# li-kunyi/dns-slam

Measured on AMD Instinct MI355X. Metric: ray-samples/s, higher is better.
Workload: dtype f32 (MLP products as 3 x f16 split-operand MFMA / 6 x bf16 for weight gradients, f32 accumulate: error <= fp32 fma chain)

## Files before the change

### dns_slam_amd/_lib.py

```python
from __future__ import annotations

import ctypes as C
import os

_HERE = os.path.dirname(os.path.abspath(__file__))
LIB_PATH = os.environ.get("DNS_HIP_LIB") or os.path.join(_HERE, "libdns_hip.so")
DNS_MAX_LEVELS = 32
ABI_VERSION = 17


class DnsGridMeta(C.Structure):
    _fields_ = [
        ("n_levels", C.c_uint32), ("n_features", C.c_uint32), ("log2_hashmap_size", C.c_uint32),
        ("base_resolution", C.c_uint32), ("total_rows", C.c_uint32), ("per_level_scale", C.c_float),
        ("scale", C.c_float * DNS_MAX_LEVELS), ("resolution", C.c_uint32 * DNS_MAX_LEVELS),
        ("size", C.c_uint32 * DNS_MAX_LEVELS), ("offset", C.c_uint32 * DNS_MAX_LEVELS),
        ("hashed", C.c_uint32 * DNS_MAX_LEVELS),
    ]


class DnsSplitRows(C.Structure):
    _fields_ = [("rows", C.c_void_p), ("exps", C.c_void_p), ("ld", C.c_uint32), ("lo_off", C.c_uint32)]


class DnsAdamTensor(C.Structure):
    _fields_ = [("p", C.c_void_p), ("g", C.c_void_p), ("m", C.c_void_p), ("v", C.c_void_p), ("n", C.c_uint64),
                ("lr", C.c_float)]


_P = C.c_void_p
_U = C.c_uint32
_I = C.c_int


class DnsTrackFused(C.Structure):
    _fields_ = [("color", _P), ("depth", _P), ("label", _P),
                ("H", C.c_int32), ("W", C.c_int32), ("H0", C.c_int32), ("H1", C.c_int32), ("W0", C.c_int32), ("W1", C.c_int32),
                ("cam", _P), ("bound", _P),
                ("pix", _P), ("t_uniform", _P), ("t_surf", _P), ("t_zero", _P), ("dmax", _P), ("iter", _P), ("n_iters", _U),
                ("n_uniform", _U), ("n_surface", _U), ("n_rays", _U),
                ("quat", _P), ("trans", _P),
                ("table", _P), ("meta", C.POINTER(DnsGridMeta)), ("n_bins", _U),
                ("w_coarse", _P), ("w_color", _P), ("w_logit", _P),
                ("n_neurons", _U), ("n_hidden_layers", _U), ("hidden", _U), ("n_feat", _U), ("n_class", _U),
                ("code", _P), ("code_dim", _U),
                ("lambda_p", C.c_float), ("lambda_d", C.c_float), ("lambda_l", C.c_float),
                ("ws", _P), ("adam_m", _P), ("adam_v", _P), ("adam_state", _P),
                ("lr_quat", C.c_float), ("lr_trans", C.c_float), ("beta1", C.c_float), ("beta2", C.c_float), ("eps", C.c_float),
                ("best_loss", _P), ("best_cam", _P), ("out", _P), ("g_quat", _P), ("g_trans", _P)]

SIGNATURES = {
# ... 40 lines not shown
    "dns_class_slots": (C.c_int, [_P, _U, _U, _I, _P, _U, _P, _P]),
    "dns_feature_block": (C.c_int, [_P, _U, _U, _P, _U, _P, _P, _U, _U, _P, _U, _P, _P]),
    "dns_rgb_sigmoid": (C.c_int, [_P, _U, _P]),
    "dns_raw_bwd": (C.c_int, [_P, _P, _U, _P, _P, _U, _I, _P]),
    "dns_lattice_points": (C.c_int, [_P, _P, _U, _P, _U, _P, _P]),
    "dns_draw_finish": (C.c_int, [_P, _P, _P, _P, _P, _P, _P, _P, _U, _U, _U, _U, _P, _P, _P, _P]),
    "dns_track_mask": (C.c_int, [_P, _P, _U, C.c_float, _P, _P]),
    "dns_keep_best": (C.c_int, [_P, _P, _P, _P, _P, _P]),
    "dns_force_half": (C.c_int, [_P, _U, _U, _P]),
    "dns_track_fused_ws_floats": (C.c_uint64, [C.POINTER(DnsTrackFused)]),
    "dns_track_fused_begin": (C.c_int, [_P, _U, _U, _P, _I, _I, _I, _I, _P, _U, _P, _P]),
    "dns_track_fused_iter": (C.c_int, [C.POINTER(DnsTrackFused), _P]),
    "dns_feature_gather": (C.c_int, [_P, _P, _P, _P, _U, _U, _U, _I, _I, _I, _I, _P, _P, _P]),
    "dns_feature_gather_frames": (C.c_int, [_P, _P, _P, _P, _P, _U, _U, _U, _U, _I, _I, _I, _I, _P, _U, _P, _P]),
    "dns_refer_poses": (C.c_int, [_P, _P, _P, _P, _U, _P, _P, _P]),
    "dns_merge_dy": (C.c_int, [_P, _U, _U, _U, _U, _P, _P, _U, _U, _P, _P]),
    "dns_add_ref_sum": (C.c_int, [_P, _U, _U, _U, _P, _P]),
    "dns_tv_fwd": (C.c_int, [_P, _U, _U, _U, _I, _U, _P, _P]),
    "dns_tv_bwd": (C.c_int, [_P, _U, _U, _U, _I, _U, _P, _P, _P]),
    "dns_group_slots": (C.c_int, [_P, _U, _U, _U, _U, _P, _P, _P, _P]),
    "dns_group_scatter": (C.c_int, [_P, _U, _U, _P, _U, _P, _P]),
    "dns_device_error": (C.c_int, [C.c_int]),
    "dns_adam_step": (C.c_int, [C.POINTER(DnsAdamTensor), _U, C.c_float, C.c_float, C.c_float, _P, _P]),
    "dns_composite_fwd": (C.c_int, [_P, _P, _P, _U, _U, _U, _P, _P, _P, _P, _P, _P]),
    "dns_composite_bwd": (C.c_int, [_P, _P, _P, _U, _U, _U, _P, _P, _P, _P, _P, _P, _P, _P]),
    "dns_mc_ws_bytes": (C.c_uint64, [_U, _U, _U]),
    "dns_mc_count": (C.c_int, [_P, _U, _U, _U, C.c_float, _P, _P, _P]),
    "dns_mc_emit": (C.c_int, [_P, _U, _U, _U, C.c_float, C.POINTER(C.c_double), C.POINTER(C.c_double), _P, _P, C.c_uint64, _P,
                              C.c_uint64, _P]),
    "dns_keyframe_project": (C.c_int, [_P, _U, _P, _U, _P, _P, _I, _I, C.POINTER(C.c_float), _P, _P, _P]),
    "dns_mesh_cc_ws_bytes": (C.c_uint64, [_U]),
    "dns_mesh_components": (C.c_int, [_P, _U, _P, _U, _P, _P, _P, _P, _P]),
    "dns_nearest_ws_bytes": (C.c_uint64, [_U, _U]),
    "dns_nearest_points": (C.c_int, [_P, _U, _P, _U, _U, _U, _P, _P, _P, _P, _P]),
    "dns_icp_ws_bytes": (C.c_uint64, [_U, _U]),
    "dns_icp_point_to_point": (C.c_int, [_P, _U, _P, _U, C.POINTER(C.c_double), C.c_float, _U, C.c_double, C.c_double, _U, _P, _P,
                                         _P, _P]),
    "dns_frustum_seen": (C.c_int, [_P, _U, _P, _U, _I, _I, C.POINTER(C.c_float), _P, _P]),
    "dns_ms_ssim_window": (None, [C.POINTER(C.c_float)]),
    "dns_ms_ssim_ws_bytes": (C.c_uint64, [_U, _U, _U]),
    "dns_ms_ssim": (C.c_int, [_P, _P, _P, _U, _U, _U, _P, _P, _P, _P, _P, _P]),
    "dns_label_confusion": (C.c_int, [_P, _P, _U, C.c_uint64, _U, _P, _P, _P]),
}


def _load():
# ... 68 lines not shown
```

### dns_slam_amd/csrc/adam.hip

```cpp
#include "common.hpp"

namespace dns {

constexpr int ADAM_MAX_TENSORS = 32;

struct AdamBatch {
  float* p[ADAM_MAX_TENSORS];
  const float* g[ADAM_MAX_TENSORS];
  float* m[ADAM_MAX_TENSORS];
  float* v[ADAM_MAX_TENSORS];
  uint32_t block_end[ADAM_MAX_TENSORS];
  uint32_t n[ADAM_MAX_TENSORS];
  float lr[ADAM_MAX_TENSORS];
  uint32_t n_tensors;
};

__global__ void adam_tick_kernel(float* __restrict__ state, float beta1, float beta2) {
  if (threadIdx.x == 0 && blockIdx.x == 0) {
    const float t = state[0] + 1.0f;
    state[0] = t;
    state[1] = 1.0f - powf(beta1, t);
    state[2] = 1.0f - powf(beta2, t);
  }
}

__global__ __launch_bounds__(256) void adam_step_kernel(AdamBatch b, const float* __restrict__ state, float beta1, float beta2,
                                                        float eps) {
  uint32_t t = 0;
  while (t + 1 < b.n_tensors && blockIdx.x >= b.block_end[t]) ++t;
  const uint32_t first = t ? b.block_end[t - 1] : 0u;
  const uint32_t i0 = (blockIdx.x - first) * 1024u + threadIdx.x * 4u;
  const uint32_t n = b.n[t];
  if (i0 >= n) return;
  const float bc1 = state[1], bc2 = state[2];
  const float step_size = b.lr[t] / bc1;
  const float inv_sqrt_bc2 = 1.0f / sqrtf(bc2);
  float* __restrict__ p = b.p[t];
  const float* __restrict__ g = b.g[t];
  float* __restrict__ m = b.m[t];
  float* __restrict__ v = b.v[t];
  const float ob1 = 1.0f - beta1, ob2 = 1.0f - beta2;
  if (i0 + 3u < n && (((uintptr_t)(p + i0) | (uintptr_t)(g + i0) | (uintptr_t)(m + i0) | (uintptr_t)(v + i0)) & 15u) == 0) {
    const float4 g4 = *reinterpret_cast<const float4*>(g + i0);
    float4 m4 = *reinterpret_cast<const float4*>(m + i0), v4 = *reinterpret_cast<const float4*>(v + i0);
    float4 p4 = *reinterpret_cast<const float4*>(p + i0);
    const float ge[4] = {g4.x, g4.y, g4.z, g4.w};
    float me[4] = {m4.x, m4.y, m4.z, m4.w}, ve[4] = {v4.x, v4.y, v4.z, v4.w}, pe[4] = {p4.x, p4.y, p4.z, p4.w};
#pragma unroll
    for (int e = 0; e < 4; ++e) {
      me[e] = beta1 * me[e] + ob1 * ge[e];
      ve[e] = beta2 * ve[e] + ob2 * ge[e] * ge[e];
      const float denom = sqrtf(ve[e]) * inv_sqrt_bc2 + eps;
      pe[e] -= step_size * (me[e] / denom);
    }
    *reinterpret_cast<float4*>(m + i0) = make_float4(me[0], me[1], me[2], me[3]);
    *reinterpret_cast<float4*>(v + i0) = make_float4(ve[0], ve[1], ve[2], ve[3]);
    *reinterpret_cast<float4*>(p + i0) = make_float4(pe[0], pe[1], pe[2], pe[3]);
    return;
  }
#pragma unroll
  for (uint32_t e = 0; e < 4; ++e) {
    const uint32_t i = i0 + e;
    if (i < n) {
      const float gi = g[i];
      const float mi = beta1 * m[i] + ob1 * gi;
      const float vi = beta2 * v[i] + ob2 * gi * gi;
      m[i] = mi;
      v[i] = vi;
      const float denom = sqrtf(vi) * inv_sqrt_bc2 + eps;
      p[i] -= step_size * (mi / denom);
    }
  }
}

}

using namespace dns;

extern "C" int dns_adam_step(const DnsAdamTensor* tensors, uint32_t n_tensors, float beta1, float beta2, float eps,
                             float* state, void* stream) {
  DNS_REQUIRE(tensors && state, "dns_adam_step: NULL argument");
  DNS_REQUIRE(n_tensors <= ADAM_MAX_TENSORS, "dns_adam_step: at most %d tensors per call (got %u)", ADAM_MAX_TENSORS, n_tensors);
  AdamBatch b;
  uint32_t nb = 0, k = 0;
  for (uint32_t i = 0; i < n_tensors; ++i) {
    if (!tensors[i].g || tensors[i].n == 0) continue;
    DNS_REQUIRE(tensors[i].p && tensors[i].m && tensors[i].v, "dns_adam_step: tensor %u has a NULL buffer", i);
    DNS_REQUIRE(tensors[i].n < (1ull << 32), "dns_adam_step: tensor %u too large", i);
    b.p[k] = tensors[i].p; b.g[k] = tensors[i].g; b.m[k] = tensors[i].m; b.v[k] = tensors[i].v;
    b.n[k] = (uint32_t)tensors[i].n;
    b.lr[k] = tensors[i].lr;
    nb += (uint32_t)((tensors[i].n + 1023) / 1024);
    b.block_end[k] = nb;
    ++k;
  }
  b.n_tensors = k;
  hipStream_t st = (hipStream_t)stream;
  DNS_LAUNCH(adam_tick_kernel, dim3(1), dim3(64), 0, st, state, beta1, beta2);
  if (k) DNS_LAUNCH(adam_step_kernel, dim3(nb), dim3(256), 0, st, b, state, beta1, beta2, eps);
  return check_launch("dns_adam_step");
}
```

### dns_slam_amd/csrc/mlp_split.hpp

```cpp
#pragma once
#include "common.hpp"
#include "split_rows.hpp"

namespace dns {
namespace sp {

typedef float f32x16 __attribute__((ext_vector_type(16)));
typedef _Float16 half8 __attribute__((ext_vector_type(8)));
typedef _Float16 half4v __attribute__((ext_vector_type(4)));

using sr::TGT_EXP;
using sr::scale_exp;

struct Frag {
  half8 hi, lo;
};

__device__ __forceinline__ uint32_t acc_row(uint32_t r, uint32_t h) { return (r & 3u) + 8u * (r >> 2) + 4u * h; }

__device__ __forceinline__ f32x16 zero16() {
  f32x16 z;
#pragma unroll
  for (int i = 0; i < 16; ++i) z[i] = 0.f;
  return z;
// ... 73 lines not shown
                                                 uint32_t lane) {
  return reinterpret_cast<const uint4*>(img) + ((rt * nsteps + s) * 2u + part) * 64u + lane;
}

template <int PREC>
__device__ __forceinline__ Frag load_frag(const _Float16* img, uint32_t nsteps, uint32_t rt, uint32_t s, uint32_t lane) {
  Frag f;
  const uint4 hi = *frag_ptr(img, nsteps, rt, s, 0, lane);
  f.hi = *reinterpret_cast<const half8*>(&hi);
  if (PREC == 3) {
    const uint4 lo = *frag_ptr(img, nsteps, rt, s, 1, lane);
    f.lo = *reinterpret_cast<const half8*>(&lo);
  } else {
    f.lo = f.hi;
  }
  return f;
}

template <int MAXQ>
struct ImgQuads {
  float4 v[MAXQ];
};

template <int MAXQ>
__device__ __forceinline__ float image_load(ImgQuads<MAXQ>& q, const float* __restrict__ M, uint32_t R, uint32_t C, uint32_t ld = 0) {
  if (ld == 0) ld = C;
  const uint32_t qpr = C >> 2, nq = R * qpr;
  const bool vec = ((((uintptr_t)M) & 15u) == 0) && ((ld & 3u) == 0);
  float m = 0.f;
  bool bad = false;
#pragma unroll
  for (int j = 0; j < MAXQ; ++j) {
    const uint32_t e = threadIdx.x + j * blockDim.x;
    q.v[j] = make_float4(0.f, 0.f, 0.f, 0.f);
    if (e < nq) {
      const uint32_t rr = e / qpr;
      const float* src = M + (size_t)rr * ld + (size_t)(e - rr * qpr) * 4u;
      if (vec) q.v[j] = *reinterpret_cast<const float4*>(src);
      else q.v[j] = make_float4(src[0], src[1], src[2], src[3]);
    }
    const float a = fmaxf(fmaxf(fabsf(q.v[j].x), fabsf(q.v[j].y)), fmaxf(fabsf(q.v[j].z), fabsf(q.v[j].w)));
    m = fmaxf(m, a);
    bad = bad || !(a < INFINITY);
  }
  return bad ? INFINITY : m;
}

template <int MAXQ>
__device__ __forceinline__ void image_scatter(const ImgQuads<MAXQ>& q, _Float16* __restrict__ img, uint32_t R, uint32_t C,
                                              bool transpose, uint32_t row_tiles, uint32_t nsteps, int kmap, float scale) {
  auto slot = [&](uint32_t i, uint32_t k, uint32_t& idx) -> bool {
    const uint32_t s = k >> 4, qq = k & 15u;
    uint32_t h, j;
    if (kmap == K_NAT) {
      h = qq >> 3;
      j = qq & 7u;
    } else {
      h = (qq >> 2) & 1u;
      j = ((qq >> 3) << 2) | (qq & 3u);
    }
    const uint32_t rt = i >> 5;
    if (rt >= row_tiles || s >= nsteps) return false;
    idx = ((((rt * nsteps + s) * 2u) * 64u) + (i & 31u) + 32u * h) * 8u + j;
    return true;
  };
  const uint32_t qpr = C >> 2, nq = R * qpr;
#pragma unroll
  for (int jq = 0; jq < MAXQ; ++jq) {
    const uint32_t e = threadIdx.x + jq * blockDim.x;
    if (e >= nq) continue;
    const uint32_t rr = e / qpr, cc = (e - rr * qpr) * 4u;
    const float vv[4] = {q.v[jq].x * scale, q.v[jq].y * scale, q.v[jq].z * scale, q.v[jq].w * scale};
    _Float16 hi[4], lo[4];
#pragma unroll
    for (int c = 0; c < 4; ++c) {
      hi[c] = (_Float16)vv[c];
      lo[c] = (_Float16)(vv[c] - (float)hi[c]);
    }
    uint32_t idx;
    if (!transpose) {
      if (slot(rr, cc, idx)) {
        half4v h4, l4;
#pragma unroll
        for (int c = 0; c < 4; ++c) { h4[c] = hi[c]; l4[c] = lo[c]; }
        *reinterpret_cast<half4v*>(img + idx) = h4;
        *reinterpret_cast<half4v*>(img + idx + 64u * 8u) = l4;
      }
    } else {
#pragma unroll
      for (uint32_t c = 0; c < 4u; ++c) {
        if (slot(cc + c, rr, idx)) {
          img[idx] = hi[c];
          img[idx + 64u * 8u] = lo[c];
        }
      }
    }
  }
}

__device__ __forceinline__ void lds_zero16(void* p, uint32_t bytes) {
  uint4* q = reinterpret_cast<uint4*>(p);
  for (uint32_t e = threadIdx.x; e < bytes / 16u; e += blockDim.x) q[e] = make_uint4(0u, 0u, 0u, 0u);
}

__device__ __forceinline__ void images_copy_in(unsigned char* lds, const unsigned char* __restrict__ src, uint32_t bytes,
                                               const unsigned char* __restrict__ exps, int* wexp) {
  const uint4* __restrict__ s4 = reinterpret_cast<const uint4*>(src);
  uint4* d4 = reinterpret_cast<uint4*>(lds);
  const uint32_t n = bytes / 16u, stride = blockDim.x;
  uint32_t e = threadIdx.x;
  for (; e + 7u * stride < n; e += 8u * stride) {
    uint4 v[8];
#pragma unroll
    for (int k = 0; k < 8; ++k) v[k] = s4[e + k * stride];
#pragma unroll
    for (int k = 0; k < 8; ++k) d4[e + k * stride] = v[k];
  }
  for (; e < n; e += stride) d4[e] = s4[e];
  if (threadIdx.x < 3) wexp[threadIdx.x] = reinterpret_cast<const int*>(exps)[threadIdx.x];
// ... 940 lines not shown
```

### dns_slam_amd/fused_step.py

```python
from __future__ import annotations

import ctypes as C
import os

import torch

from . import ops
from ._lib import DnsAdamTensor, DnsSplitRows, DnsTrackFused, check, ptr
from .common import get_quad_from_c2w, get_rotation_from_quad

_V = C.c_void_p


def _morton2(row, col):
    def spread(v):
        v = v & 0xffff
        v = (v | (v << 8)) & 0x00ff00ff
        v = (v | (v << 4)) & 0x0f0f0f0f
        v = (v | (v << 2)) & 0x33333333
        return (v | (v << 1)) & 0x55555555
    return spread(col) | (spread(row) << 1)


class _Set:
    pass


class MapStep:
    def __init__(self, mapper, target_frames, quad_list=None, T_list=None, prep=None, features=None, lambda_lt=10.0,
                 smooth=True, betas=(0.9, 0.999), eps=1e-8, keep_hidden=False, split_rows=None, refer_frames=None):
        m = self.m = mapper
# ... 120 lines not shown
        if self.half:
            self.xh = torch.empty(P, ld, device=dev, dtype=torch.float16)
            self.feath = torch.empty(P, self.n_feat, device=dev, dtype=torch.float16)
        self.use_prep = (bool(getattr(m, "prepared_images", os.environ.get("DNS_PREPARED_IMAGES", "1") != "0")) and not self.sr
                         and not self.half)
        self._blobs, self._prep_jobs = {}, []
        if self.use_prep:
            raw_lib = ops.lib._raw
            G = int(self.p_pool.shape[0]) if self.p_pool.dim() == 2 else 1
            live_n = (self.live >> 16) & 0xff
            jobs = [(self.p_coarse, self.shp_c, self.shp_c[1], 1, 0, 0),
                    (self.p_coarse, self.shp_c, 1, 1, 0, 0),
                    (self.p_pool, self.shp_f, self.shp_f[1], G, int(self.p_pool.shape[-1]), 0),
                    (self.p_color, self.shp_col, self.shp_col[1], 1, 0, self.live),
                    (self.p_logit, self.shp_log, self.shp_log[1], 1, 0, self.live)]
            for prm, shp_, n_out, n_sets, stride, lv in jobs:
                n_in_eff = live_n if lv else shp_[0]
                nfl = int(raw_lib.dns_mlp_prepared_floats(n_in_eff, n_out, shp_[2], shp_[3]))
                blob = torch.empty(nfl * n_sets + 64, device=dev)
                off = (-blob.data_ptr() // 4) % 4
                view = blob[off:off + nfl * n_sets]
                self._blobs[(prm.data_ptr(), n_out)] = view
                self._prep_jobs.append((prm, shp_[0], n_out, shp_[2], shp_[3], n_sets, stride, view, lv, blob))
        self.sr_planes = 1 if self.fp16 else 2
        self.sr_flags = 1 if self.fp16 else 0
        if self.sr:
            np_ = self.sr_planes
            h16 = lambda *s_: torch.empty(*s_, device=dev, dtype=torch.float16)
            i32 = lambda n_: torch.empty(n_, device=dev, dtype=torch.int32)
            self.xs, self.xexp = h16(P, np_ * ld), i32(P)
            self.fxs, self.fexp = h16(P, np_ * self.n_feat), i32(P)
            self.rows_x = DnsSplitRows(self.xs.data_ptr(), self.xexp.data_ptr(), np_ * ld, ld if np_ == 2 else 0)
            self.rows_f = DnsSplitRows(self.fxs.data_ptr(), self.fexp.data_ptr(), np_ * self.n_feat, self.n_feat if np_ == 2 else 0)
        nf = self.hid + 1
        self.coarse = f(P, nf)
        n_groups = self.n_groups = max(len(pool), 1)
        self.n_slots = (P + 127) // 128 * 128 + 128 * n_groups
        self.group_ws = torch.empty(512, device=dev, dtype=torch.int32)
        self.feat = f(P, self.n_feat)
        self.slot = torch.empty(P, device=dev, dtype=torch.int64)
        self.sets = []
        for _ in range(2):
            st_ = _Set()
            o_G = (P * nf + 3) // 4 * 4
            st_.zb = torch.zeros(o_G + n_G, device=dev)
            st_.fine, st_.G = st_.zb[:P * nf].view(P, nf), st_.zb[o_G:]
# ... 96 lines not shown

            code = spread(ii.reshape(-1)) | (spread(jj.reshape(-1)) << 1) | (spread(kk.reshape(-1)) << 2)
            self.lat_order_l = torch.argsort(code).contiguous()
            self.lat_order = elem[self.lat_order_l].to(torch.int32).contiguous()
            self.lat_slot = torch.empty_like(self.lat_order_l)
            self.lat_slot[self.lat_order_l] = torch.arange(Pl, device=dev)
            self.occ_x, self.d_occ_x = f(Pl, 1), f(Pl, 1)
            _, c_vox, c_off, c_mar = m._lattice_consts
            self.lat_consts = (C.c_double * 9)(*[float(v) for t in (c_vox, c_off, c_mar) for v in t.cpu().tolist()])
            self.tv = f(1)
            self.w_sm = torch.full((1,), m.lambda_sm if self.union else m.lambda_sm / self.world, device=dev)
            self.ws_mlp_l = mlp_ws(Pl, self.shp_c)
            self.h_l = f(self.shp_c[3] * Pl * self.shp_c[2]) if self.keep_h_lat else None
            self.ws_enc_l = enc_ws(Pl)
        if getattr(m, "_side_stream", None) is None:
            m._side_stream = torch.cuda.Stream(device=dev)
        self.side = m._side_stream
        self.steps = 0

    def _prepare_weights(self, st):
        for prm, n_in, n_out, nn, nl, n_sets, stride, view, lv, _ in self._prep_jobs:
            check(ops.lib.dns_mlp_prepare(ptr(prm), n_in, n_out, nn, nl, n_sets, stride, ptr(view), lv, st), "dns_mlp_prepare")

    def _w(self, params, n_out):
        blob = self._blobs.get((params.data_ptr(), n_out)) if self.use_prep else None
        if blob is None:
            return ptr(params), 0
        return ptr(blob), ops.MLP_PREPARED_FLAG

    def _lattice_branch(self, cur, st):
        lib = ops.lib
        Pl, ld, pe = self.Pl, self.ld, self.pe_dim
        pts = self.pts_l
        check(lib.dns_lattice_points(ptr(cur.draws["r6"]), self.lat_consts, self.n_lat, ptr(self.lat_order), Pl, ptr(pts), st),
              "dns_lattice_points")
        meta = C.byref(self.meta.c)
        grid_l = _V(self.bufl.data_ptr() + 4 * pe)
        n_in, _, nn, nl = self.shp_c
        if self.half:
            check(lib.dns_encode_fwd_split(ptr(pts), None, Pl, self.n_bins, ptr(self.p_table), meta, None, None, 0, ptr(self.xhl), ld,
                                           None, ops.SPLIT_PLAIN, None, st), "dns_encode_fwd_split")
            check(lib.dns_mlp_fwd_half(ptr(self.xhl), ld, None, 0, 0, ptr(self.p_coarse), n_in, 1, nn, nl, ptr(self.occ), 1, Pl,
                                       None, None, 0, 0, st), "dns_mlp_fwd_half")
        elif self.sr:
            check(lib.dns_encode_fwd_split(ptr(pts), None, Pl, self.n_bins, ptr(self.p_table), meta, None, ptr(self.bufl), ld,
                                           ptr(self.xsl), self.sr_planes * ld, ptr(self.xexpl), self.sr_flags, None, st), "dns_encode_fwd_split")
# ... 78 lines not shown
                                  ptr(self.slot), stream), "dns_class_slots")
        check(lib.dns_group_slots(ptr(self.slot), P, self.n_groups, 2, self.n_slots, ptr(self.group_ws), ptr(st_.row_index),
                                  ptr(st_.tile_group), stream), "dns_group_slots")
        st_.zb.zero_()

    @torch.no_grad()
    def step(self, draws=None, last=False):
        m, lib = self.m, ops.lib
        if torch.cuda.is_current_stream_capturing():
            self._captured = True
        main = torch.cuda.current_stream()
        st = _V(main.cuda_stream)
        K, npf, N, S, P, ld, pe = self.K, self.npf, self.N, self.S, self.P, self.ld, self.pe_dim
        prefetch = getattr(m, "prefetch_draws", False) and draws is None
        cur = self.sets[self.steps % 2]
        if not prefetch or cur.ev is None:
            self._prepare(cur, st, draws)
        else:
            main.wait_event(cur.ev)
        cur.ev = None
        self.cur = cur
        pix, (t_surf, t_zero) = cur.draws["pix"], cur.draws["jitter"]
        on_side = self.smooth and getattr(m, "overlap_smooth", False)
        if on_side or prefetch:
            self.side.wait_stream(main)
        prep_ev = None
        if self.use_prep:
            if on_side or prefetch:
                with torch.cuda.stream(self.side):
                    self._prepare_weights(_V(self.side.cuda_stream))
                    prep_ev = torch.cuda.Event()
                    prep_ev.record(self.side)
            else:
                self._prepare_weights(st)
        if on_side:
            with torch.cuda.stream(self.side):
                self._lattice_branch(cur, _V(self.side.cuda_stream))
        elif self.smooth:
            self._lattice_branch(cur, st)
        if prefetch and not last:
            nxt = self.sets[(self.steps + 1) % 2]
            with torch.cuda.stream(self.side):
                self._prepare(nxt, _V(self.side.cuda_stream), None)
                nxt.ev = torch.cuda.Event()
                nxt.ev.record(self.side)
            for t in (nxt.draws["pix"], nxt.draws["jitter"][0], nxt.draws["jitter"][1], nxt.dmax):
                t.record_stream(main)

        jstride = self.ns if t_surf.dim() == 2 else 0
        prep = self.prep
# ... 169 lines not shown
            with torch.cuda.stream(self.side):
                st2 = _V(self.side.cuda_stream)
                check(lib.dns_encode_bwd(ptr(self.x3), self.b6, P, self.n_bins, ptr(self.p_table), meta, ptr(self.d_buf), ld, d_grid,
                                         ld, None, ptr(self.d_x3), ptr(self.dydx), None, 0, 0, st2), "dns_encode_bwd")
                if self.stem:
                    check(lib.dns_add_ref_sum(ptr(self.d_rel), self.R, self.Pf, P, ptr(self.d_x3), st2), "dns_add_ref_sum")
                check(lib.dns_raygen_bwd(ptr(pix), ptr(self.Q), self.camv, 0, H, 0, W, K, npf, S, ptr(self.z), ptr(self.d_x3), None,
                                         None, ptr(self.ray_ws), ptr(cur.g_quat), ptr(cur.g_trans), st2), "dns_raygen_bwd")
        check(lib.dns_encode_bwd(ptr(self.x3), self.b6, P, self.n_bins, ptr(self.p_table), meta, ptr(self.d_buf), ld, d_grid, ld,
                                 ptr(cur.g_table), ptr(self.d_x3) if (self.is_BA and not fork_pose) else None, ptr(self.dydx),
                                 ptr(self.ws_enc), self.scatter_form, self.scatter_cap, st), "dns_encode_bwd")
        if self.is_BA and not fork_pose:
            if self.stem:
                check(lib.dns_add_ref_sum(ptr(self.d_rel), self.R, self.Pf, P, ptr(self.d_x3), st), "dns_add_ref_sum")
            check(lib.dns_raygen_bwd(ptr(pix), ptr(self.Q), self.camv, 0, H, 0, W, K, npf, S, ptr(self.z), ptr(self.d_x3), None,
                                     None, ptr(self.ray_ws), ptr(cur.g_quat), ptr(cur.g_trans), st), "dns_raygen_bwd")
        if on_side:
            main.wait_stream(self.side)
        if self.dist_on:
            import torch.distributed as dist
            work2 = dist.all_reduce(cur.G_late, op=dist.ReduceOp.SUM, group=m.dist.group, async_op=True)
            work.wait()
            work2.wait()
        check(lib.dns_adam_step(cur.adam_items, self.n_adam, self.betas[0], self.betas[1], self.eps, ptr(self.adam_state), st),
              "dns_adam_step")
        self.steps += 1

    def set_lambda_lt(self, value):
        if getattr(self, "_captured", False) and float(value) != float(self.lam[3]):
            raise RuntimeError("MapStep.set_lambda_lt: the step has been captured into a hipGraph -- the loss weights are kernel "
                               "arguments frozen at capture time; capture one graph per weight schedule phase")
        self.lam[3] = float(value)

    g_table = property(lambda self: self.cur.g_table)
    g_coarse = property(lambda self: self.cur.g_coarse)
    g_color = property(lambda self: self.cur.g_color)
    g_logit = property(lambda self: self.cur.g_logit)
    g_pool = property(lambda self: self.cur.g_pool)
    g_merge = property(lambda self: self.cur.g_merge)
    g_quat = property(lambda self: self.cur.g_quat)
    g_trans = property(lambda self: self.cur.g_trans)

    def losses(self):
        t = self.out
        terms = {"p_loss": t[0], "d_loss": t[1], "l_loss": t[2], "lt_loss": t[3], "fs_loss": t[4], "opacity_loss": t[5]}
        total = t[6]
        if self.smooth:
            terms["smooth_loss"] = self.tv[0]
# ... 386 lines not shown
```

### include/dns_hip.h

```cpp
#ifndef DNS_HIP_H
#define DNS_HIP_H

#include <stdint.h>

#ifdef __cplusplus
extern "C" {
#endif

#define DNS_ABI_VERSION 17
#define DNS_MAX_LEVELS 32

#define DNS_OK 0
#define DNS_E_ARG (-1)
#define DNS_E_LAUNCH (-2)
#define DNS_E_STATE (-3)

typedef struct DnsGridMeta {
  uint32_t n_levels;
  uint32_t n_features;
  uint32_t log2_hashmap_size;
  uint32_t base_resolution;
  uint32_t total_rows;
  float per_level_scale;
  float scale[DNS_MAX_LEVELS];
  uint32_t resolution[DNS_MAX_LEVELS];
  uint32_t size[DNS_MAX_LEVELS];
  uint32_t offset[DNS_MAX_LEVELS];
  uint32_t hashed[DNS_MAX_LEVELS];
} DnsGridMeta;

int dns_abi_version(void);
const char* dns_last_error(void);
// ... 138 lines not shown
                      const float* sums, float* out, void* stream);
int dns_loss_bwd(const float* lambdas, uint32_t N, uint32_t S, uint32_t C, uint32_t L, int tracker,
                 const float* out, const float* g_total, const float* pred_color, const float* pred_depth,
                 const float* pred_var, const float* pred_logits, const float* gt_color, const float* gt_depth,
                 const int64_t* gt_label, const uint8_t* valid, const float* fine, const float* coarse, const float* z,
                 float* d_color, float* d_depth, float* d_var, float* d_logits, float* d_fine, float* d_coarse,
                 uint32_t ldd_fine, void* stream);

int dns_loss_bwd_points(const float* lambdas, uint32_t N, uint32_t S, uint32_t C, uint32_t L, const float* out,
                        const float* g_total, const float* gt_depth, const uint8_t* valid, const float* fine, const float* coarse,
                        const float* z, float* d_fine, float* d_coarse, uint32_t ldd_fine, const float* d_occ, uint32_t ld_occ,
                        void* stream);

typedef struct DnsAdamTensor {
  float* p;
  const float* g;
  float* m;
  float* v;
  uint64_t n;
  float lr;
} DnsAdamTensor;
int dns_adam_step(const DnsAdamTensor* tensors, uint32_t n_tensors, float beta1, float beta2, float eps,
                  float* state, void* stream);

typedef struct DnsTrackFused {
  const float* color;
  const float* depth;
  const float* label;
  int32_t H, W, H0, H1, W0, W1;
  const double* cam;
  const double* bound;
  const int64_t* pix;
  const float* t_uniform;
  const float* t_surf;
  const float* t_zero;
  const uint32_t* dmax;
  uint32_t* iter;
  uint32_t n_iters;
  uint32_t n_uniform, n_surface, n_rays;
  float* quat;
  float* trans;
  const float* table;
  const DnsGridMeta* meta;
  uint32_t n_bins;
  const float* w_coarse;
  const float* w_color;
// ... 112 lines not shown
```

Measured before the change: 169.8 million.

## Fuse MLP weight image preparation into the Adam step kernel

The Adam update kernel now also rebuilds the split f16 hi/lo MFMA weight images for MLP tensors. The last block to finish each tensor, found through an atomic counter, computes the block scale exponents and scatters the forward and backward images. This removes the separate dns_mlp_prepare launches at the start of each step, which now run only when a parameter's version changes outside the optimizer. In exchange a single block serially writes all images for a tensor at the tail of the kernel, and the bias-correction tick moves into a last-block atomic.

```diff
diff --git a/dns_slam_amd/_lib.py b/dns_slam_amd/_lib.py
--- a/dns_slam_amd/_lib.py
+++ b/dns_slam_amd/_lib.py
@@ -6,7 +6,7 @@
 _HERE = os.path.dirname(os.path.abspath(__file__))
 LIB_PATH = os.environ.get("DNS_HIP_LIB") or os.path.join(_HERE, "libdns_hip.so")
 DNS_MAX_LEVELS = 32
-ABI_VERSION = 17
+ABI_VERSION = 18
 
 
 class DnsGridMeta(C.Structure):
@@ -27,6 +27,14 @@
     _fields_ = [("p", C.c_void_p), ("g", C.c_void_p), ("m", C.c_void_p), ("v", C.c_void_p), ("n", C.c_uint64),
                 ("lr", C.c_float)]
 
+
+class DnsAdamImage(C.Structure):
+    _fields_ = [("images", C.c_void_p), ("tensor", C.c_uint32), ("n_in", C.c_uint32), ("n_out", C.c_uint32),
+                ("n_neurons", C.c_uint32), ("n_hidden_layers", C.c_uint32), ("live_in", C.c_uint32), ("n_sets", C.c_uint32),
+                ("param_stride", C.c_uint32)]
+
+
+ADAM_WORK_WORDS = 33
 
 _P = C.c_void_p
 _U = C.c_uint32
@@ -113,6 +121,8 @@
     "dns_group_scatter": (C.c_int, [_P, _U, _U, _P, _U, _P, _P]),
     "dns_device_error": (C.c_int, [C.c_int]),
     "dns_adam_step": (C.c_int, [C.POINTER(DnsAdamTensor), _U, C.c_float, C.c_float, C.c_float, _P, _P]),
+    "dns_adam_step_images": (C.c_int, [C.POINTER(DnsAdamTensor), _U, C.POINTER(DnsAdamImage), _U, C.c_float, C.c_float, C.c_float,
+                                       _P, _P, _P]),
     "dns_composite_fwd": (C.c_int, [_P, _P, _P, _U, _U, _U, _P, _P, _P, _P, _P, _P]),
     "dns_composite_bwd": (C.c_int, [_P, _P, _P, _U, _U, _U, _P, _P, _P, _P, _P, _P, _P, _P]),
     "dns_mc_ws_bytes": (C.c_uint64, [_U, _U, _U]),
diff --git a/dns_slam_amd/csrc/adam.hip b/dns_slam_amd/csrc/adam.hip
--- a/dns_slam_amd/csrc/adam.hip
+++ b/dns_slam_amd/csrc/adam.hip
@@ -1,4 +1,5 @@
 #include "common.hpp"
+#include "mlp_split.hpp"
 
 namespace dns {
 
@@ -24,15 +25,11 @@
   }
 }
 
-__global__ __launch_bounds__(256) void adam_step_kernel(AdamBatch b, const float* __restrict__ state, float beta1, float beta2,
-                                                        float eps) {
-  uint32_t t = 0;
-  while (t + 1 < b.n_tensors && blockIdx.x >= b.block_end[t]) ++t;
-  const uint32_t first = t ? b.block_end[t - 1] : 0u;
-  const uint32_t i0 = (blockIdx.x - first) * 1024u + threadIdx.x * 4u;
+__device__ __forceinline__ void adam_update_block(const AdamBatch& b, uint32_t t, uint32_t blk, float bc1, float bc2, float beta1,
+                                                  float beta2, float eps) {
+  const uint32_t i0 = blk * 1024u + threadIdx.x * 4u;
   const uint32_t n = b.n[t];
   if (i0 >= n) return;
-  const float bc1 = state[1], bc2 = state[2];
   const float step_size = b.lr[t] / bc1;
   const float inv_sqrt_bc2 = 1.0f / sqrtf(bc2);
   float* __restrict__ p = b.p[t];
@@ -73,6 +70,133 @@
   }
 }
 
+__device__ __forceinline__ uint32_t adam_tensor_of_block(const AdamBatch& b, uint32_t blk) {
+  uint32_t t = 0;
+  while (t + 1 < b.n_tensors && blk >= b.block_end[t]) ++t;
+  return t;
+}
+
+__global__ __launch_bounds__(256) void adam_step_kernel(AdamBatch b, const float* __restrict__ state, float beta1, float beta2,
+                                                        float eps) {
+  const uint32_t t = adam_tensor_of_block(b, blockIdx.x);
+  const uint32_t first = t ? b.block_end[t - 1] : 0u;
+  adam_update_block(b, t, blockIdx.x - first, state[1], state[2], beta1, beta2, eps);
+}
+
+constexpr int ADAM_MAX_IMAGES = 8;
+
+struct AdamImage {
+  unsigned char* blob;
+  uint32_t n_in_w, n_live, n_out, nn, nl;
+  uint32_t n_sets, param_stride, blob_stride;
+  uint32_t f_h, f_out, f_exp, ns0, mt_f;
+  uint32_t b_base, b_h, b_outT, b_hT, b_inT, b_exp, nch, mt_b;
+};
+struct AdamImages {
+  AdamImage d[ADAM_MAX_IMAGES];
+  int8_t of_tensor[ADAM_MAX_TENSORS][2];
+};
+
+__device__ __forceinline__ float4 adam_load_quad(const float* src, bool vec) {
+  if (vec) return *reinterpret_cast<const float4*>(src);
+  return make_float4(src[0], src[1], src[2], src[3]);
+}
+
+__device__ __forceinline__ void adam_write_images(const AdamImage& d, const float* p, float* red, int* wexp) {
+  const uint32_t nn = d.nn, nt = nn >> 5, nsh = nn >> 4;
+  const uint32_t qpr_in = d.n_live >> 2, nq_in = nn * qpr_in;
+  const uint32_t qpr_h = nn >> 2, nq_h = (d.nl - 1u) * nn * qpr_h, nq_out = d.n_out * qpr_h;
+  for (uint32_t set = 0; set < d.n_sets; ++set) {
+    const float* w_in = p + (size_t)set * d.param_stride;
+    const float* w_h = w_in + nn * d.n_in_w;
+    const float* w_out = w_h + (d.nl - 1u) * nn * nn;
+    const bool vec_in = ((((uintptr_t)w_in) & 15u) == 0) && ((d.n_in_w & 3u) == 0);
+    const bool vec_h = (((uintptr_t)w_h) & 15u) == 0, vec_out = (((uintptr_t)w_out) & 15u) == 0;
+    float m[3] = {0.f, 0.f, 0.f};
+    bool bad[3] = {false, false, false};
+    for (uint32_t e = threadIdx.x; e < nq_in; e += 256u) {
+      const uint32_t rr = e / qpr_in;
+      sp::quad_absmax(adam_load_quad(w_in + (size_t)rr * d.n_in_w + (e - rr * qpr_in) * 4u, vec_in), m[0], bad[0]);
+    }
+    for (uint32_t e = threadIdx.x; e < nq_h; e += 256u) sp::quad_absmax(adam_load_quad(w_h + e * 4u, vec_h), m[1], bad[1]);
+    for (uint32_t e = threadIdx.x; e < nq_out; e += 256u) sp::quad_absmax(adam_load_quad(w_out + e * 4u, vec_out), m[2], bad[2]);
+    sp::block_scale_exps(bad[0] ? INFINITY : m[0], bad[1] ? INFINITY : m[1], bad[2] ? INFINITY : m[2], red, wexp);
+    const float s_in = sp::pow2f(wexp[0]), s_h = sp::pow2f(wexp[1]), s_out = sp::pow2f(wexp[2]);
+    unsigned char* fwd = d.blob + (size_t)set * d.blob_stride;
+    unsigned char* bwd = fwd + d.b_base;
+    _Float16* f_in = reinterpret_cast<_Float16*>(fwd);
+    _Float16* f_h = reinterpret_cast<_Float16*>(fwd + d.f_h);
+    _Float16* f_out = reinterpret_cast<_Float16*>(fwd + d.f_out);
+    _Float16* b_in = reinterpret_cast<_Float16*>(bwd);
+    _Float16* b_h = reinterpret_cast<_Float16*>(bwd + d.b_h);
+    _Float16* b_outT = reinterpret_cast<_Float16*>(bwd + d.b_outT);
+    _Float16* b_hT = reinterpret_cast<_Float16*>(bwd + d.b_hT);
+    _Float16* b_inT = reinterpret_cast<_Float16*>(bwd + d.b_inT);
+    for (uint32_t e = threadIdx.x; e < nq_in; e += 256u) {
+      const uint32_t rr = e / qpr_in, cc = (e - rr * qpr_in) * 4u;
+      const float4 q = adam_load_quad(w_in + (size_t)rr * d.n_in_w + cc, vec_in);
+      sp::image_put_quad(f_in, q, rr, cc, false, nt, d.ns0, sp::K_NAT, s_in);
+      sp::image_put_quad(b_in, q, rr, cc, false, nt, 2u * d.nch, sp::K_NAT, s_in);
+      sp::image_put_quad(b_inT, q, rr, cc, true, d.nch, nsh, sp::K_CHAIN, s_in);
+    }
+    for (uint32_t e = threadIdx.x; e < nq_h; e += 256u) {
+      const uint32_t rr = e / qpr_h, cc = (e - rr * qpr_h) * 4u;
+      const float4 q = adam_load_quad(w_h + e * 4u, vec_h);
+      sp::image_put_quad(f_h, q, rr, cc, false, nt, nsh, sp::K_CHAIN, s_h);
+      sp::image_put_quad(b_h, q, rr, cc, false, nt, nsh, sp::K_CHAIN, s_h);
+      sp::image_put_quad(b_hT, q, rr, cc, true, nt, nsh, sp::K_CHAIN, s_h);
+    }
+    for (uint32_t e = threadIdx.x; e < nq_out; e += 256u) {
+      const uint32_t rr = e / qpr_h, cc = (e - rr * qpr_h) * 4u;
+      const float4 q = adam_load_quad(w_out + e * 4u, vec_out);
+      sp::image_put_quad(f_out, q, rr, cc, false, d.mt_f, nsh, sp::K_CHAIN, s_out);
+      sp::image_put_quad(b_outT, q, rr, cc, true, nt, 2u * d.mt_b, sp::K_NAT, s_out);
+    }
+    if (threadIdx.x < 4u) {
+      const int ex = threadIdx.x < 3u ? wexp[threadIdx.x] : 0;
+      reinterpret_cast<int*>(fwd + d.f_exp)[threadIdx.x] = ex;
+      reinterpret_cast<int*>(bwd + d.b_exp)[threadIdx.x] = ex;
+    }
+    __syncthreads();
+  }
+}
+
+__global__ __launch_bounds__(256) void adam_step_images_kernel(AdamBatch b, AdamImages im, float* state, uint32_t* work, float beta1,
+                                                               float beta2, float eps) {
+  __shared__ float red[12];
+  __shared__ int wexp[4];
+  __shared__ uint32_t last;
+  const uint32_t t = adam_tensor_of_block(b, blockIdx.x);
+  const uint32_t first = t ? b.block_end[t - 1] : 0u;
+  const float tt = state[0] + 1.0f;
+  const float bc1 = 1.0f - powf(beta1, tt), bc2 = 1.0f - powf(beta2, tt);
+  adam_update_block(b, t, blockIdx.x - first, bc1, bc2, beta1, beta2, eps);
+  if (im.of_tensor[t][0] >= 0) {
+    __threadfence();
+    __syncthreads();
+    if (threadIdx.x == 0) last = (atomicAdd(&work[1u + t], 1u) + 1u == b.block_end[t] - first) ? 1u : 0u;
+    __syncthreads();
+    if (last) {
+      __threadfence();
+      if (threadIdx.x == 0) work[1u + t] = 0u;
+#pragma unroll 1
+      for (int k = 0; k < 2; ++k) {
+        const int di = im.of_tensor[t][k];
+        if (di >= 0) adam_write_images(im.d[di], b.p[t], red, wexp);
+      }
+    }
+  }
+  __syncthreads();
+  if (threadIdx.x == 0) {
+    if (atomicAdd(&work[0], 1u) + 1u == gridDim.x) {
+      work[0] = 0u;
+      state[0] = tt;
+      state[1] = bc1;
+      state[2] = bc2;
+    }
+  }
+}
+
 }
 
 using namespace dns;
@@ -100,3 +224,76 @@
   if (k) DNS_LAUNCH(adam_step_kernel, dim3(nb), dim3(256), 0, st, b, state, beta1, beta2, eps);
   return check_launch("dns_adam_step");
 }
+
+static bool adam_image_layout(AdamImage& d) {
+  const uint32_t nt = d.nn / 32u, frag = 2048u, nsh = d.nn / 16u, hid = (d.nl - 1u) * nt * nsh * frag;
+  d.ns0 = (d.n_live + 15u) / 16u;
+  d.mt_f = (d.n_out + 31u) / 32u;
+  d.f_h = nt * d.ns0 * frag;
+  d.f_out = d.f_h + hid;
+  d.f_exp = d.f_out + d.mt_f * nsh * frag;
+  d.b_base = d.f_exp + 16u;
+  d.nch = d.n_live <= 32u ? 1u : (d.n_live <= 96u ? 3u : 4u);
+  d.mt_b = d.n_out <= 32u ? 1u : 2u;
+  d.b_h = nt * 2u * d.nch * frag;
+  d.b_outT = d.b_h + hid;
+  d.b_hT = d.b_outT + nt * 2u * d.mt_b * frag;
+  d.b_inT = d.b_hT + hid;
+  d.b_exp = d.b_inT + d.nch * nsh * frag;
+  d.blob_stride = d.b_base + d.b_exp + 16u;
+  return d.b_base == mlp_prepared_fwd_bytes(d.n_live, d.n_out, d.nn, d.nl) && d.blob_stride == mlp_prepared_bytes(d.n_live, d.n_out, d.nn, d.nl);
+}
+
+extern "C" int dns_adam_step_images(const DnsAdamTensor* tensors, uint32_t n_tensors, const DnsAdamImage* images, uint32_t n_images,
+                                    float beta1, float beta2, float eps, float* state, uint32_t* work, void* stream) {
+  DNS_REQUIRE(tensors && state && work && (images || n_images == 0), "dns_adam_step_images: NULL argument");
+  DNS_REQUIRE(n_tensors <= ADAM_MAX_TENSORS, "dns_adam_step_images: at most %d tensors per call (got %u)", ADAM_MAX_TENSORS, n_tensors);
+  DNS_REQUIRE(n_images <= ADAM_MAX_IMAGES, "dns_adam_step_images: at most %d images per call (got %u)", ADAM_MAX_IMAGES, n_images);
+  AdamBatch b;
+  AdamImages im;
+  for (int i = 0; i < ADAM_MAX_TENSORS; ++i) im.of_tensor[i][0] = im.of_tensor[i][1] = -1;
+  uint32_t order[ADAM_MAX_TENSORS], no = 0;
+  for (int pass = 0; pass < 2; ++pass)
+    for (uint32_t i = 0; i < n_tensors; ++i) {
+      bool has = false;
+      for (uint32_t j = 0; j < n_images; ++j) has = has || images[j].tensor == i;
+      if (has == (pass == 0)) order[no++] = i;
+    }
+  uint32_t nb = 0, k = 0;
+  for (uint32_t oi = 0; oi < n_tensors; ++oi) {
+    const uint32_t i = order[oi];
+    if (!tensors[i].g || tensors[i].n == 0) continue;
+    DNS_REQUIRE(tensors[i].p && tensors[i].m && tensors[i].v, "dns_adam_step_images: tensor %u has a NULL buffer", i);
+    DNS_REQUIRE(tensors[i].n < (1ull << 32), "dns_adam_step_images: tensor %u too large", i);
+    b.p[k] = tensors[i].p; b.g[k] = tensors[i].g; b.m[k] = tensors[i].m; b.v[k] = tensors[i].v;
+    b.n[k] = (uint32_t)tensors[i].n;
+    b.lr[k] = tensors[i].lr;
+    nb += (uint32_t)((tensors[i].n + 1023) / 1024);
+    b.block_end[k] = nb;
+    uint32_t cnt = 0;
+    for (uint32_t j = 0; j < n_images; ++j) {
+      const DnsAdamImage& s = images[j];
+      if (s.tensor != i) continue;
+      DNS_REQUIRE(cnt < 2, "dns_adam_step_images: at most two images per tensor (tensor %u)", i);
+      AdamImage& d = im.d[j];
+      d.blob = reinterpret_cast<unsigned char*>(s.images);
+      d.n_in_w = s.n_in; d.n_live = s.live_in ? s.live_in : s.n_in; d.n_out = s.n_out; d.nn = s.n_neurons; d.nl = s.n_hidden_layers;
+      d.n_sets = s.n_sets; d.param_stride = s.n_sets > 1 ? s.param_stride : 0u;
+      DNS_REQUIRE(d.blob && (((uintptr_t)d.blob) % 16) == 0, "dns_adam_step_images: image %u: NULL or not 16-byte aligned", j);
+      DNS_REQUIRE((d.nn == 32 || d.nn == 64) && (d.nl == 1 || d.nl == 2) && d.n_in_w % 4 == 0 && d.n_in_w <= 128 && d.n_out >= 1 &&
+                      d.n_out <= 64 && d.n_live % 8 == 0 && d.n_live >= 8 && d.n_live <= d.n_in_w && d.n_sets >= 1,
+                  "dns_adam_step_images: image %u: unsupported shape in=%u live=%u out=%u neurons=%u layers=%u", j, d.n_in_w, d.n_live,
+                  d.n_out, d.nn, d.nl);
+      DNS_REQUIRE(adam_image_layout(d), "dns_adam_step_images: image %u: layout does not match dns_mlp_prepared_floats", j);
+      const uint64_t view = (uint64_t)d.nn * d.n_in_w + (uint64_t)(d.nl - 1) * d.nn * d.nn + (uint64_t)d.n_out * d.nn;
+      DNS_REQUIRE((uint64_t)(d.n_sets - 1) * d.param_stride + view <= tensors[i].n, "dns_adam_step_images: image %u reaches past tensor %u", j, i);
+      im.of_tensor[k][cnt++] = (int8_t)j;
+    }
+    ++k;
+  }
+  b.n_tensors = k;
+  hipStream_t st = (hipStream_t)stream;
+  if (k) DNS_LAUNCH(adam_step_images_kernel, dim3(nb), dim3(256), 0, st, b, im, state, work, beta1, beta2, eps);
+  else DNS_LAUNCH(adam_tick_kernel, dim3(1), dim3(64), 0, st, state, beta1, beta2);
+  return check_launch("dns_adam_step_images");
+}
diff --git a/dns_slam_amd/csrc/mlp_split.hpp b/dns_slam_amd/csrc/mlp_split.hpp
--- a/dns_slam_amd/csrc/mlp_split.hpp
+++ b/dns_slam_amd/csrc/mlp_split.hpp
@@ -119,6 +119,12 @@
   float4 v[MAXQ];
 };
 
+__device__ __forceinline__ void quad_absmax(const float4& q, float& m, bool& bad) {
+  const float a = fmaxf(fmaxf(fabsf(q.x), fabsf(q.y)), fmaxf(fabsf(q.z), fabsf(q.w)));
+  m = fmaxf(m, a);
+  bad = bad || !(a < INFINITY);
+}
+
 template <int MAXQ>
 __device__ __forceinline__ float image_load(ImgQuads<MAXQ>& q, const float* __restrict__ M, uint32_t R, uint32_t C, uint32_t ld = 0) {
   if (ld == 0) ld = C;
@@ -136,62 +142,67 @@
       if (vec) q.v[j] = *reinterpret_cast<const float4*>(src);
       else q.v[j] = make_float4(src[0], src[1], src[2], src[3]);
     }
-    const float a = fmaxf(fmaxf(fabsf(q.v[j].x), fabsf(q.v[j].y)), fmaxf(fabsf(q.v[j].z), fabsf(q.v[j].w)));
-    m = fmaxf(m, a);
-    bad = bad || !(a < INFINITY);
+    quad_absmax(q.v[j], m, bad);
   }
   return bad ? INFINITY : m;
+}
+
+__device__ __forceinline__ bool image_slot(uint32_t i, uint32_t k, uint32_t row_tiles, uint32_t nsteps, int kmap, uint32_t& idx) {
+  const uint32_t s = k >> 4, qq = k & 15u;
+  uint32_t h, j;
+  if (kmap == K_NAT) {
+    h = qq >> 3;
+    j = qq & 7u;
+  } else {
+    h = (qq >> 2) & 1u;
+    j = ((qq >> 3) << 2) | (qq & 3u);
+  }
+  const uint32_t rt = i >> 5;
+  if (rt >= row_tiles || s >= nsteps) return false;
+  idx = ((((rt * nsteps + s) * 2u) * 64u) + (i & 31u) + 32u * h) * 8u + j;
+  return true;
+}
+constexpr uint32_t IMG_LO_OFF = 64u * 8u;
+
+__device__ __forceinline__ void image_put_quad(_Float16* __restrict__ img, const float4& q, uint32_t rr, uint32_t cc, bool transpose,
+                                               uint32_t row_tiles, uint32_t nsteps, int kmap, float scale) {
+  const float vv[4] = {q.x * scale, q.y * scale, q.z * scale, q.w * scale};
+  _Float16 hi[4], lo[4];
+#pragma unroll
+  for (int c = 0; c < 4; ++c) {
+    hi[c] = (_Float16)vv[c];
+    lo[c] = (_Float16)(vv[c] - (float)hi[c]);
+  }
+  uint32_t idx;
+  if (!transpose) {
+    if (image_slot(rr, cc, row_tiles, nsteps, kmap, idx)) {
+      half4v h4, l4;
+#pragma unroll
+      for (int c = 0; c < 4; ++c) { h4[c] = hi[c]; l4[c] = lo[c]; }
+      *reinterpret_cast<half4v*>(img + idx) = h4;
+      *reinterpret_cast<half4v*>(img + idx + IMG_LO_OFF) = l4;
+    }
+  } else {
+#pragma unroll
+    for (uint32_t c = 0; c < 4u; ++c) {
+      if (image_slot(cc + c, rr, row_tiles, nsteps, kmap, idx)) {
+        img[idx] = hi[c];
+        img[idx + IMG_LO_OFF] = lo[c];
+      }
+    }
+  }
 }
 
 template <int MAXQ>
 __device__ __forceinline__ void image_scatter(const ImgQuads<MAXQ>& q, _Float16* __restrict__ img, uint32_t R, uint32_t C,
                                               bool transpose, uint32_t row_tiles, uint32_t nsteps, int kmap, float scale) {
-  auto slot = [&](uint32_t i, uint32_t k, uint32_t& idx) -> bool {
-    const uint32_t s = k >> 4, qq = k & 15u;
-    uint32_t h, j;
-    if (kmap == K_NAT) {
-      h = qq >> 3;
-      j = qq & 7u;
-    } else {
-      h = (qq >> 2) & 1u;
-      j = ((qq >> 3) << 2) | (qq & 3u);
-    }
-    const uint32_t rt = i >> 5;
-    if (rt >= row_tiles || s >= nsteps) return false;
-    idx = ((((rt * nsteps + s) * 2u) * 64u) + (i & 31u) + 32u * h) * 8u + j;
-    return true;
-  };
   const uint32_t qpr = C >> 2, nq = R * qpr;
 #pragma unroll
   for (int jq = 0; jq < MAXQ; ++jq) {
     const uint32_t e = threadIdx.x + jq * blockDim.x;
     if (e >= nq) continue;
     const uint32_t rr = e / qpr, cc = (e - rr * qpr) * 4u;
-    const float vv[4] = {q.v[jq].x * scale, q.v[jq].y * scale, q.v[jq].z * scale, q.v[jq].w * scale};
-    _Float16 hi[4], lo[4];
-#pragma unroll
-    for (int c = 0; c < 4; ++c) {
-      hi[c] = (_Float16)vv[c];
-      lo[c] = (_Float16)(vv[c] - (float)hi[c]);
-    }
-    uint32_t idx;
-    if (!transpose) {
-      if (slot(rr, cc, idx)) {
-        half4v h4, l4;
-#pragma unroll
-        for (int c = 0; c < 4; ++c) { h4[c] = hi[c]; l4[c] = lo[c]; }
-        *reinterpret_cast<half4v*>(img + idx) = h4;
-        *reinterpret_cast<half4v*>(img + idx + 64u * 8u) = l4;
-      }
-    } else {
-#pragma unroll
-      for (uint32_t c = 0; c < 4u; ++c) {
-        if (slot(cc + c, rr, idx)) {
-          img[idx] = hi[c];
-          img[idx + 64u * 8u] = lo[c];
-        }
-      }
-    }
+    image_put_quad(img, q.v[jq], rr, cc, transpose, row_tiles, nsteps, kmap, scale);
   }
 }
 
diff --git a/dns_slam_amd/fused_step.py b/dns_slam_amd/fused_step.py
--- a/dns_slam_amd/fused_step.py
+++ b/dns_slam_amd/fused_step.py
@@ -6,7 +6,7 @@
 import torch
 
 from . import ops
-from ._lib import DnsAdamTensor, DnsSplitRows, DnsTrackFused, check, ptr
+from ._lib import ADAM_WORK_WORDS, DnsAdamImage, DnsAdamTensor, DnsSplitRows, DnsTrackFused, check, ptr
 from .common import get_quad_from_c2w, get_rotation_from_quad
 
 _V = C.c_void_p
@@ -173,6 +173,21 @@
                 view = blob[off:off + nfl * n_sets]
                 self._blobs[(prm.data_ptr(), n_out)] = view
                 self._prep_jobs.append((prm, shp_[0], n_out, shp_[2], shp_[3], n_sets, stride, view, lv, blob))
+        self.adam_images = self.use_prep and bool(getattr(m, "adam_images", os.environ.get("DNS_ADAM_IMAGES", "1") != "0"))
+        self._img_versions = None
+        if self.adam_images:
+            tensor_of = {it[0].data_ptr(): k for k, it in enumerate(items)}
+            jobs_ = [j for j in self._prep_jobs if j[0].data_ptr() in tensor_of and j[5] >= 1]
+            if len(jobs_) != len(self._prep_jobs):
+                self.adam_images = False
+        if self.adam_images:
+            self._adam_imgs = (DnsAdamImage * len(jobs_))()
+            for d, (prm, n_in, n_out, nn, nl, n_sets, stride, view, lv, _) in zip(self._adam_imgs, jobs_):
+                d.images, d.tensor = view.data_ptr(), tensor_of[prm.data_ptr()]
+                d.n_in, d.n_out, d.n_neurons, d.n_hidden_layers = n_in, n_out, nn, nl
+                d.live_in, d.n_sets, d.param_stride = (lv >> 16) & 0xff, n_sets, stride
+            self.adam_work = torch.zeros(ADAM_WORK_WORDS, device=dev, dtype=torch.int32)
+            self._img_params = [j[0] for j in jobs_]
         self.sr_planes = 1 if self.fp16 else 2
         self.sr_flags = 1 if self.fp16 else 0
         if self.sr:
@@ -315,6 +330,15 @@
         for prm, n_in, n_out, nn, nl, n_sets, stride, view, lv, _ in self._prep_jobs:
             check(ops.lib.dns_mlp_prepare(ptr(prm), n_in, n_out, nn, nl, n_sets, stride, ptr(view), lv, st), "dns_mlp_prepare")
 
+    def invalidate_images(self):
+        self._img_versions = None
+
+    def _refresh_images(self, st):
+        ver = [p_._version for p_ in self._img_params]
+        if ver != self._img_versions:
+            self._prepare_weights(st)
+            self._img_versions = ver
+
     def _w(self, params, n_out):
         blob = self._blobs.get((params.data_ptr(), n_out)) if self.use_prep else None
         if blob is None:
@@ -439,10 +463,12 @@
         self.cur = cur
         pix, (t_surf, t_zero) = cur.draws["pix"], cur.draws["jitter"]
         on_side = self.smooth and getattr(m, "overlap_smooth", False)
+        if self.adam_images:
+            self._refresh_images(st)
         if on_side or prefetch:
             self.side.wait_stream(main)
         prep_ev = None
-        if self.use_prep:
+        if self.use_prep and not self.adam_images:
             if on_side or prefetch:
                 with torch.cuda.stream(self.side):
                     self._prepare_weights(_V(self.side.cuda_stream))
@@ -658,8 +684,13 @@
             work2 = dist.all_reduce(cur.G_late, op=dist.ReduceOp.SUM, group=m.dist.group, async_op=True)
             work.wait()
             work2.wait()
-        check(lib.dns_adam_step(cur.adam_items, self.n_adam, self.betas[0], self.betas[1], self.eps, ptr(self.adam_state), st),
-              "dns_adam_step")
+        if self.adam_images:
+            check(lib.dns_adam_step_images(cur.adam_items, self.n_adam, self._adam_imgs, len(self._adam_imgs), self.betas[0],
+                                           self.betas[1], self.eps, ptr(self.adam_state), ptr(self.adam_work), st),
+                  "dns_adam_step_images")
+        else:
+            check(lib.dns_adam_step(cur.adam_items, self.n_adam, self.betas[0], self.betas[1], self.eps, ptr(self.adam_state), st),
+                  "dns_adam_step")
         self.steps += 1
 
     def set_lambda_lt(self, value):
diff --git a/include/dns_hip.h b/include/dns_hip.h
--- a/include/dns_hip.h
+++ b/include/dns_hip.h
@@ -7,7 +7,7 @@
 extern "C" {
 #endif
 
-#define DNS_ABI_VERSION 17
+#define DNS_ABI_VERSION 18
 #define DNS_MAX_LEVELS 32
 
 #define DNS_OK 0
@@ -192,6 +192,16 @@
 } DnsAdamTensor;
 int dns_adam_step(const DnsAdamTensor* tensors, uint32_t n_tensors, float beta1, float beta2, float eps,
                   float* state, void* stream);
+#define DNS_ADAM_WORK_WORDS 33
+typedef struct DnsAdamImage {
+  void* images;
+  uint32_t tensor;
+  uint32_t n_in, n_out, n_neurons, n_hidden_layers;
+  uint32_t live_in;
+  uint32_t n_sets, param_stride;
+} DnsAdamImage;
+int dns_adam_step_images(const DnsAdamTensor* tensors, uint32_t n_tensors, const DnsAdamImage* images, uint32_t n_images,
+                         float beta1, float beta2, float eps, float* state, uint32_t* work, void* stream);
 
 typedef struct DnsTrackFused {
   const float* color;
```

Measured after the change: 93.03 million. -45.2%, worse.
